# pymc-devs/pymc

Measured on AMD Instinct MI355X. Metric: effective samples/sec (and leapfrog steps/sec), 10k-param hierarchical logistic regression, one NUTS chain per GPU, higher is better.
Workload: dtype f64

## Files before the change

pymc_amd/csrc/engine.hip:

```cpp
#include <hip/hip_runtime.h>

#include <algorithm>
#include <atomic>
#include <chrono>
#include <cmath>
#include <cstdio>
#include <cstdlib>
#include <cstring>
#include <mutex>
#include <thread>
#include <utility>
#include <ctime>
#include <string>
#include <vector>

#include "kernels.h"
#include "small_kernel.h"
#include "mixture_kernel.h"
#include "nuts_mi355.h"
#include "pcg64_stream.h"
#include "advi.h"

static thread_local std::string g_err;

// ... 1185 lines not shown
  const int n = m->md.n, D = lg.D, SPAN = WAVE * m->rows_rpl;
  const int64_t n_tiles = tile0[lg.G];
  lg.ga = 1; lg.ga_w = gpw ? GB_W : W;
  lg.ga_gpw = gpw;
  lg.ga_bsz = gpw ? gpw : (lg.G + 31) / 32;
  lg.ga_flags = env_int("NUTS_GA_FLAGS", 0);
  lg.ga_T_uni = 0; lg.ga_ng_uni = 0;
  {
    bool uni = lg.G > 0;
    for (int g = 1; g < lg.G; ++g) uni = uni && (gptr[g + 1] - gptr[g] == gptr[1] - gptr[0]);
    if (uni && maxT > 0) { lg.ga_T_uni = (int32_t)maxT; lg.ga_ng_uni = gptr[1] - gptr[0]; }
  }
  lg.ga_nblk = (lg.G + lg.ga_bsz - 1) / lg.ga_bsz;
  lg.ga_auxel = n - lg.G * D;
  lg.ga_naux = m->ga_struct_ok == 2 ? (lg.ga_auxel + WAVE * lg.ga_w - 1) / (WAVE * lg.ga_w) : 0;
  lg.ga_nrec = lg.ga_nblk + lg.ga_naux;
  bool ones0 = D == 8 && env_int("NUTS_GA_ONES0", 1) != 0 && lg.N > 0;
  for (int64_t i = 0; ones0 && i < lg.N; ++i) ones0 = s->rows_X[i * D] == 1.0;
  const int DX = ones0 ? D - 1 : D;
  lg.ga_dx = DX;
  const int64_t TS = (int64_t)DX * SPAN, GA_SKEW = env_int("NUTS_GA_SKEW", DX == 7 || DX == 5 ? 1120 : 1056);
  if (GA_SKEW % DX != 0) return refuse("NUTS_GA_SKEW must be a multiple of the stored column count");
  std::vector<int64_t> coff((size_t)lg.G * W, 0);
  int64_t pos = 0, max_ct = 0;
  for (int g = 0; g < lg.G; ++g) {
    const int64_t T = tile0[g + 1] - tile0[g];
    for (int w = 0; w < W; ++w) {
      const int64_t ct = (int64_t)(w + 1) * T / W - (int64_t)w * T / W;
      coff[(size_t)g * W + w] = pos;
      pos += ct * TS + GA_SKEW;
      max_ct = std::max(max_ct, ct);
    }
  }
  lg.ga_cstride_uni = 0;
  if (lg.ga_T_uni > 0 && lg.ga_T_uni % W == 0) {
    lg.ga_cstride_uni = (lg.ga_T_uni / W) * TS + GA_SKEW;
  } else lg.ga_T_uni = 0;
  lg.Npad = n_tiles * SPAN; lg.n_spans = n_tiles;
  std::vector<double> xt((size_t)(pos + TS), 0.0);
  std::vector<int8_t> yy((size_t)(pos / DX + 2 * SPAN), 0);
  for (int g = 0; g < lg.G; ++g) {
    const int64_t T = tile0[g + 1] - tile0[g];
    for (int64_t i = gptr[g]; i < gptr[g + 1]; ++i) {
      const int64_t r = i - gptr[g], t = r / SPAN, rr = r % SPAN;
      int w = (int)(((t + 1) * W - 1) / std::max<int64_t>(T, 1));
      while (w > 0 && (int64_t)w * T / W > t) --w;
      while (w + 1 < W && (int64_t)(w + 1) * T / W <= t) ++w;
      const int64_t base = coff[(size_t)g * W + w] + (t - (int64_t)w * T / W) * TS;
      for (int d = D - DX; d < D; ++d) xt[(size_t)(base + (int64_t)(d - (D - DX)) * SPAN + rr)] = s->rows_X[i * D + d];
      yy[(size_t)(base / DX + rr)] = s->rows_y[i];
    }
  }
  lg.Xt = m->keep(dev_upload(xt.data(), xt.size()));
  lg.y = m->keep(dev_upload(yy.data(), yy.size()));
  m->rows_xt_len = (int64_t)xt.size(); m->rows_y_len = (int64_t)yy.size();
  lg.ga_coff = m->keep(dev_upload(coff.data(), coff.size()));
  lg.ga_tile0 = m->keep(dev_upload(tile0.data(), tile0.size()));
  lg.ga_part = m->keep(dev_alloc<double>((size_t)lg.G * PART_STRIDE));
  const size_t bpart_len = gpw ? 2 * (size_t)PART_STRIDE * ((lg.ga_nrec + WAVE - 1) / WAVE * WAVE) : 2 * (size_t)lg.ga_nrec * PART_STRIDE;
  lg.ga_bpart = m->keep(dev_alloc<double>(bpart_len));
  lg.ga_ticket = m->keep(dev_alloc<unsigned>(lg.ga_nblk));
  if (lg.ga_part) hipMemset(lg.ga_part, 0, (size_t)lg.G * PART_STRIDE * sizeof(double));
  if (lg.ga_bpart) hipMemset(lg.ga_bpart, 0, bpart_len * sizeof(double));
  if (lg.ga_ticket) hipMemset(lg.ga_ticket, 0, lg.ga_nblk * sizeof(unsigned));
  m->rows_grid = gpw ? lg.ga_nblk : lg.G;
  return true;
}

static bool build_rows_spans(nuts_model* m, const nuts_model_spec* s, int cus) {
  RowsDev& lg = m->md.lg;
// ... 941 lines not shown
extern "C" nuts_group* nuts_group_create(void) {
  nuts_group* g = new nuts_group();
  if (hipStreamCreateWithFlags(&g->stream, hipStreamNonBlocking) != hipSuccess) { g_err = "nuts_group_create: no stream"; delete g; return nullptr; }
  return g;
}

extern "C" int nuts_group_add(nuts_group* g, nuts_chain* c) {
  if (!g || !c || !c->m) return NUTS_E_ARG;
  nuts_model* m = c->m;
  const MvnDev& mv = m->md.mv;
  if (m->group) { g_err = "nuts_group_add: the chain's model already belongs to a group"; return NUTS_E_ARG; }
  if (m->n_chains != 1) { g_err = "nuts_group_add: a member model carries exactly one chain (its launch parity and records are the chain's)"; return NUTS_E_ARG; }
  const RowsDev& lg = m->md.lg;
  const bool is_mvn = m->md.has_mvn && (mv.aligned == 4 || mv.aligned == 8);
  const bool is_rows = m->md.has_logit && !m->md.has_mvn && lg.ga && lg.ga_naux == 0 && lg.D == 8 && m->ga_struct_ok == 1;
  const int rows_kind = lg.ga_gpw > 0 ? 3 : 2;
  if (!(is_mvn || is_rows) || c->dense || c->host_pot) {
    g_err = "nuts_group_add: chain groups advance models that are one constant-covariance MvNormal node on the row-aligned pass or the "
            "hierarchical-logit rows on the group-aligned pass (diagonal mass matrix); this chain is neither";
    return NUTS_E_ARG;
  }
  const int rows_lds = g->n == 0 ? env_int("NUTS_ROWS_GROUP_LDS", 1) : g->rows_lds;
  const int cap = g->n == 0 ? (is_rows ? ((rows_lds || rows_kind == 3) ? GAL_MAXC : GAM_MAXNC) : ((is_mvn && mv.aligned == 8 && mv.k % 16 == 0 && c->group_wide) ? GRP_MAXC : MVM_MAXC)) : g->cap;
  if (g->n >= cap) {
    g_err = cap == GRP_MAXC ? "nuts_group_add: a wide group holds at most 16 chains" : (cap == GAL_MAXC ? "nuts_group_add: a rows group holds at most 8 chains" : "nuts_group_add: a group holds at most 4 chains");
    return NUTS_E_ARG;
  }
  if (g->n > 0 && g->kind != (is_rows ? rows_kind : 1)) { g_err = "nuts_group_add: not the same model as the group's"; return NUTS_E_ARG; }
  HIPCHK(hipStreamSynchronize(m->stream));
  if (is_rows) {
    if (nuts_model* base = group_base(g)) {
      const RowsDev& bl = base->md.lg;
      if (bl.N != lg.N || bl.G != lg.G || bl.D != lg.D || bl.ga_dx != lg.ga_dx || bl.ga_w != lg.ga_w || bl.ga_gpw != lg.ga_gpw || bl.ga_nblk != lg.ga_nblk || bl.Npad != lg.Npad || bl.ga_T_uni != lg.ga_T_uni ||
          bl.ga_cstride_uni != lg.ga_cstride_uni || bl.ga_bsz != lg.ga_bsz || bl.ga_nrec != lg.ga_nrec || bl.sigma_tr != lg.sigma_tr ||
          bl.off_mu != lg.off_mu || bl.off_sigma != lg.off_sigma || bl.off_z != lg.off_z || base->md.n != m->md.n ||
          std::memcmp(&bl.z_np_mu, &lg.z_np_mu, 8 * sizeof(double)) != 0) {
        g_err = "nuts_group_add: not the same model as the group's"; return NUTS_E_ARG;
      }
      const size_t nx = (size_t)base->rows_xt_len, ny = (size_t)base->rows_y_len;
      if (nx != (size_t)m->rows_xt_len || ny != (size_t)m->rows_y_len) { g_err = "nuts_group_add: not the same model as the group's"; return NUTS_E_ARG; }
      const size_t slab = (size_t)1 << 22;
      std::vector<double> a(slab), b(slab);
      for (size_t o = 0; o < nx; o += slab) {
        const size_t k = std::min(slab, nx - o);
        HIPCHK(hipMemcpy(a.data(), bl.Xt + o, k * sizeof(double), hipMemcpyDeviceToHost));
        HIPCHK(hipMemcpy(b.data(), lg.Xt + o, k * sizeof(double), hipMemcpyDeviceToHost));
        if (std::memcmp(a.data(), b.data(), k * sizeof(double)) != 0) { g_err = "nuts_group_add: not the same model as the group's (the design matrices differ)"; return NUTS_E_ARG; }
      }
      std::vector<int8_t> ya(ny), yb(ny);
      HIPCHK(hipMemcpy(ya.data(), bl.y, ny, hipMemcpyDeviceToHost));
      HIPCHK(hipMemcpy(yb.data(), lg.y, ny, hipMemcpyDeviceToHost));
      if (std::memcmp(ya.data(), yb.data(), ny) != 0) { g_err = "nuts_group_add: not the same model as the group's (the observations differ)"; return NUTS_E_ARG; }
    }
  } else
  if (nuts_model* base = group_base(g)) {
    const MvnDev& bv = base->md.mv;
    if (bv.k != mv.k || bv.aligned != mv.aligned || bv.konst != mv.konst) { g_err = "nuts_group_add: not the same model as the group's"; return NUTS_E_ARG; }
    const size_t kk = (size_t)mv.k * mv.k;
    std::vector<double> a(kk + mv.k), b(kk + mv.k);
    HIPCHK(hipMemcpy(a.data(), bv.prec, kk * sizeof(double), hipMemcpyDeviceToHost));
    HIPCHK(hipMemcpy(b.data(), mv.prec, kk * sizeof(double), hipMemcpyDeviceToHost));
    HIPCHK(hipMemcpy(a.data() + kk, bv.mu, mv.k * sizeof(double), hipMemcpyDeviceToHost));
    HIPCHK(hipMemcpy(b.data() + kk, mv.mu, mv.k * sizeof(double), hipMemcpyDeviceToHost));
    if (std::memcmp(a.data(), b.data(), a.size() * sizeof(double)) != 0) { g_err = "nuts_group_add: not the same model as the group's (precision or mean differ)"; return NUTS_E_ARG; }
  }
  if (is_rows && (rows_lds || rows_kind == 3) && !g->gal_konst_dev) {
    HIPCHK(hipMalloc((void**)&g->gal_konst_dev, GAL_MAXC * sizeof(GalConst)));
// ... 1628 lines not shown
```

pymc_amd/csrc/model_dev.h:

```cpp
#pragma once
#include "device_math.h"
#include "nuts_mi355.h"

#define MAX_BTERMS 8
#define MAX_DERIVED 4
#define MAX_FACTOR_BT 6
#define MAX_DEFERRED 256
#define LOGIT_MAXD 8
#define SEG_MAIN_MAX 10

struct VarDev {
  int32_t offset, size, transform, deferred;
  double lower, upper;
  int32_t normal_prior;
  int32_t def_base;
  double np_mu, np_inv_var, np_lognorm;
};

struct Contrib {
  int32_t f;
  int16_t arg, slot;
  int32_t owner;
  int32_t fast;
  int32_t dist, pad;
// ... 13 lines not shown
  struct { int16_t arg, slot; int32_t bterm; } e[MAX_FACTOR_BT];
};

struct RowsDev {
  int64_t N, Npad;
  int32_t D, G;
  const double* Xt;
  const int8_t* y;
  const int64_t* gptr;
  int32_t off_mu, off_sigma, off_z, sigma_tr;
  int32_t var_mu, var_sigma, var_z, pad;
  int32_t def_mu, def_sigma;
  int32_t segK, seg_pad;
  int64_t n_spans;
  int32_t n_waves, n_seg;
  const int32_t* run_ptr;
  const int4* runs;
  const int32_t* gseg_ptr;
  double* seg_part;
  int32_t n_mixed, n_mixed_seg;
  const int64_t* mixed_span;
  const int32_t* mixed_g0;
  const int32_t* mixed_seg_base;
  const int32_t* gmix_ptr;
  double* mixed_part;
  double* wave_lp;
  int32_t ga, ga_w;
  int32_t ga_dx, ga_gpw;
  int32_t ga_nblk, ga_bsz;
  int32_t ga_T_uni, ga_flags;
  int64_t ga_ng_uni;
  const int32_t* ga_tile0;
  const int64_t* ga_coff;
  int64_t ga_cstride_uni;
  unsigned* ga_ticket;
  double* ga_part;
  double* ga_bpart;
  int32_t ga_naux, ga_nrec, ga_auxel, ga_pad2;
  double z_np_mu, z_np_inv_var, z_np_lognorm;
  double mu_c[3];
  double sg_c[2];
};

struct MvnDev {
  int32_t k, off;
  const double* mu;
  const double* prec;
  double konst;
  double* rowq;
  double* gdense;
  const double* winv; const double* winv_t;
  double* wy;
  int32_t aligned, al_nwg;
  double* al_part;
};

#define MIX_MAXK 16
struct MixDev {
  int64_t N;
  int32_t K, off_mu, off_sigma, off_w;
  int32_t tr_sigma, nwg;
  int32_t w_simplex, pad_;
  double alpha[MIX_MAXK], w_konst;
  const double* y;
  const double* assign;
  double sigma_c[MIX_MAXK], logw_c[MIX_MAXK];
  double* part;
// ... 89 lines not shown
  long long* ticks;
  int32_t tick_j;
  int32_t fdead_mode;
  int32_t* fdead;
  int32_t n_gsf, n_gs_elems;
  int32_t po_gsf, po_gslot;
  int32_t n_gs_blocks, n_orphans_b;
  double* gs_part;
  int32_t n_swf, sw_bytes, sw_rows, sw_po_leaf, sw_po_instr, sw_po_slot;
  int32_t sw_max_leaves, sw_max_slots, sw_max_instr, sw_blocks;
  const char* sw_blob;
  int32_t gs_lds_rows, gs_lds_bytes;
  double* adj;
  int32_t n_glong, glong_pad;
  const GLong* glong;
  double* adj_red;
  int32_t n_lins, n_lin_targets;
  const LinDev* lins;
  const LinTarget* lin_targets;
  const LinSrc* lin_srcs;
  double* lin_gdense;
};

#ifdef NUTS_KTIMING
__device__ __forceinline__ long long tick_now() {
  unsigned long long t;
  asm volatile("s_waitcnt vmcnt(0) lgkmcnt(0)\n\ts_memtime %0\n\ts_waitcnt lgkmcnt(0)" : "=s"(t) :: "memory");
  return (long long)t;
}
#define TICK(md, cond, slot) do { if (cond) (md).ticks[slot] = tick_now(); } while (0)
#else
#define TICK(md, cond, slot) do { } while (0)
#endif

__device__ __forceinline__ void st_agent(double* p, double v) {
  __hip_atomic_store(reinterpret_cast<unsigned long long*>(p), (unsigned long long)__double_as_longlong(v), __ATOMIC_RELAXED,
                     __HIP_MEMORY_SCOPE_AGENT);
}
__device__ __forceinline__ double ld_agent(const double* p) {
  return __longlong_as_double((long long)__hip_atomic_load(reinterpret_cast<const unsigned long long*>(p), __ATOMIC_RELAXED,
                                                           __HIP_MEMORY_SCOPE_AGENT));
}

template <int BATCH = 8>
__device__ __forceinline__ double sum_strided(const double* base, int stride, int s0, int s1) {
  double acc = 0.0;
  for (int s = s0; s < s1; s += BATCH) {
    double v[BATCH];
#pragma unroll
    for (int u = 0; u < BATCH; ++u) v[u] = base[(int64_t)min(s + u, s1 - 1) * stride];
#pragma unroll
    for (int u = 0; u < BATCH; ++u) acc += (s + u < s1) ? v[u] : 0.0;
  }
  return acc;
}

#define CTL_CHUNKS 8

__device__ __forceinline__ double deferred_finish(double gx_local, double S, double dxdq, double dj) {
  return fma(gx_local + S, dxdq, dj);
}

#define PROG_LDS_MAX 12288

struct Prog {
  const VarDev* vars;
// ... 778 lines not shown
```

pymc_amd/csrc/rows_ga_kernel.h:

```cpp
#pragma once
#include "rows_kernel.h"

__device__ __forceinline__ void ga_def_local(const RowsDev& R, bool is_mu, double qn, double& gx, double& dxdq, double& dj, double& lp) {
  if (is_mu) {
    const double r = qn - R.mu_c[0];
    const double z = r * R.mu_c[1];
    lp = -0.5 * z * z - R.mu_c[2] + (-0.91893853320467274178);
    gx = -z * R.mu_c[1]; dxdq = 1.0; dj = 0.0;
  } else {
    double x, lj;
    if (R.sigma_tr == NUTS_TR_LOG) { x = exp(qn); dxdq = x; lj = qn; dj = 1.0; }
    else { x = qn; dxdq = 1.0; lj = 0.0; dj = 0.0; }
    const double z = x * R.sg_c[0];
    double lpf = -0.5 * z * z - R.sg_c[1] + (-0.22579135264472743236);
    double g = -z * R.sg_c[0];
    if (!(x >= 0)) { lpf = -INFINITY; g = 0.0; }
    gx = g; lp = lj + lpf;
  }
}

template <int D, int RPL>
__device__ __forceinline__ void ga_load(const RowsDev& R, int64_t xoff, int lane, double (&x)[D][RPL], uint32_t& ybits) {
  constexpr int SPAN = WAVE * RPL;
  const double* tile = R.Xt + xoff + lane * RPL;
  const int8_t* yp = R.y + xoff / D + lane * RPL;
  if (RPL == 2) ybits = *reinterpret_cast<const uint16_t*>(yp);
  else ybits = *reinterpret_cast<const uint32_t*>(yp);
#pragma unroll
  for (int d = 0; d < D; ++d) {
#pragma unroll
    for (int k = 0; k < RPL; k += 2) {
      const double2 a = *reinterpret_cast<const double2*>(tile + d * SPAN + k);
      x[d][k] = a.x; x[d][k + 1] = a.y;
    }
  }
}

typedef double ga_v2d __attribute__((ext_vector_type(2)));
struct GaTileRegs { ga_v2d c[8]; uint32_t y; };

__device__ __forceinline__ void ga_issue8(const double* base , const int8_t* ybase,
                                          uint32_t voff16, uint32_t voff2, GaTileRegs& t) {
  const double* base2 = base + 512;
  asm volatile(
      "s_nop 4\n\t"
      "global_load_dwordx4 %0, %9, %10\n\t"
      "global_load_dwordx4 %1, %9, %10 offset:1024\n\t"
      "global_load_dwordx4 %2, %9, %10 offset:2048\n\t"
      "global_load_dwordx4 %3, %9, %10 offset:3072\n\t"
      "global_load_dwordx4 %4, %9, %11\n\t"
      "global_load_dwordx4 %5, %9, %11 offset:1024\n\t"
      "global_load_dwordx4 %6, %9, %11 offset:2048\n\t"
      "global_load_dwordx4 %7, %9, %11 offset:3072\n\t"
      "global_load_ushort %8, %12, %13"
      : "=&v"(t.c[0]), "=&v"(t.c[1]), "=&v"(t.c[2]), "=&v"(t.c[3]), "=&v"(t.c[4]), "=&v"(t.c[5]), "=&v"(t.c[6]), "=&v"(t.c[7]), "=&v"(t.y)
      : "v"(voff16), "s"(base), "s"(base2), "v"(voff2), "s"(ybase)
      : "memory");
}

template <int N>
__device__ __forceinline__ void ga_wait8(GaTileRegs& t) {
  asm volatile("s_waitcnt vmcnt(%9)"
               : "+v"(t.c[0]), "+v"(t.c[1]), "+v"(t.c[2]), "+v"(t.c[3]), "+v"(t.c[4]), "+v"(t.c[5]), "+v"(t.c[6]), "+v"(t.c[7]), "+v"(t.y)
               : "i"(N));
}

struct GaTileRegs7 { ga_v2d c[7]; uint32_t y; };

__device__ __forceinline__ void ga_issue8(const double* base, const int8_t* ybase, uint32_t voff16, uint32_t voff2, GaTileRegs7& t) {
  const double* base2 = base + 512;
  asm volatile(
      "s_nop 4\n\t"
      "global_load_dwordx4 %0, %8, %9\n\t"
      "global_load_dwordx4 %1, %8, %9 offset:1024\n\t"
      "global_load_dwordx4 %2, %8, %9 offset:2048\n\t"
      "global_load_dwordx4 %3, %8, %9 offset:3072\n\t"
      "global_load_dwordx4 %4, %8, %10\n\t"
      "global_load_dwordx4 %5, %8, %10 offset:1024\n\t"
      "global_load_dwordx4 %6, %8, %10 offset:2048\n\t"
      "global_load_ushort %7, %11, %12"
      : "=&v"(t.c[0]), "=&v"(t.c[1]), "=&v"(t.c[2]), "=&v"(t.c[3]), "=&v"(t.c[4]), "=&v"(t.c[5]), "=&v"(t.c[6]), "=&v"(t.y)
      : "v"(voff16), "s"(base), "s"(base2), "v"(voff2), "s"(ybase)
      : "memory");
}

template <int N>
__device__ __forceinline__ void ga_wait8(GaTileRegs7& t) {
  asm volatile("s_waitcnt vmcnt(%8)"
               : "+v"(t.c[0]), "+v"(t.c[1]), "+v"(t.c[2]), "+v"(t.c[3]), "+v"(t.c[4]), "+v"(t.c[5]), "+v"(t.c[6]), "+v"(t.y)
               : "i"(N));
}

__device__ __forceinline__ void ga_unpack(const GaTileRegs& t, double (&xx)[8][2]) {
#pragma unroll
  for (int dd = 0; dd < 8; ++dd) { xx[dd][0] = t.c[dd].x; xx[dd][1] = t.c[dd].y; }
}
__device__ __forceinline__ void ga_unpack(const GaTileRegs7& t, double (&xx)[8][2]) {
  xx[0][0] = 1.0; xx[0][1] = 1.0;
#pragma unroll
  for (int dd = 1; dd < 8; ++dd) { xx[dd][0] = t.c[dd - 1].x; xx[dd][1] = t.c[dd - 1].y; }
}
template <int DX> struct GaTileSel { typedef GaTileRegs type; };
template <> struct GaTileSel<7> { typedef GaTileRegs7 type; };

template <int D, int RPL, bool ILV = false>
__device__ __forceinline__ void ga_tile(const double (&x)[D][RPL], uint32_t yb, const double (&beta)[D], int nvalid, int lane,
                                        double (&acc)[D], double& lp) {
  if constexpr (ILV && RPL == 2) {
    double eta[2] = {0.0, 0.0}, yk[2], l[2], rr[2];
#pragma unroll
    for (int d = 0; d < D; ++d) { eta[0] = fma(x[d][0], beta[d], eta[0]); eta[1] = fma(x[d][1], beta[d], eta[1]); }
    yk[0] = (double)(yb & 0xffu); yk[1] = (double)((yb >> 8) & 0xffu);
    logit_row2(eta, yk, l, rr);
#pragma unroll
    for (int k = 0; k < 2; ++k) {
      const bool in = lane * 2 + k < nvalid;
      lp += in ? l[k] : 0.0;
      rr[k] = in ? rr[k] : 0.0;
    }
#pragma unroll
    for (int d = 0; d < D; ++d) { acc[d] = fma(rr[0], x[d][0], acc[d]); acc[d] = fma(rr[1], x[d][1], acc[d]); }
    return;
  }
// ... 38 lines not shown
__device__ __forceinline__ void ga_hyper(const ModelDev& md, const QView& qv, int fold, int par, int lane, double& hval0, double& hph0) {
  const RowsDev& R = md.lg;
  if (fold & GA_FOLD_SRC) {
    const LeanSrc prev = lean_src(md, par ^ 1);
    rows_hyper_fold_elem<D>(R, prev.part, prev.stride, prev.nblk, prev.def_loc, qv, lane, hval0, hph0);
  } else {
    const int e = lane % (2 * D);
    const int i = e < D ? R.off_mu + e : R.off_sigma + (e - D);
    if (qv.composed) { hph0 = qv.p_half(i); hval0 = fma(qv.eps, qv.var[i] * hph0, qv.q[i]); }
    else { hph0 = 0.0; hval0 = qv.q[i]; }
  }
}

template <int D, int RPL, int DX = D>
__global__ __launch_bounds__(64 * GA_MAXW, 4) void k_rows_ga(GaArgs a) {
  constexpr int SPAN = WAVE * RPL;
  static_assert(DX == D || (D == 8 && DX == 7), "only the intercept column of an 8-column model is elided");
  typedef typename GaTileSel<DX>::type Tile;
  constexpr int LOADS = DX + 1;
  const ModelDev& md = a.md;
  const ArenaDev& A = a.A;
  const EvalIO& io = a.io;
  const int j = a.j, rev = a.rev, fold = a.fold, par = a.par, d = a.d, max_depth = a.max_depth;
  const double Emax = a.Emax;
  HostStatus* const st = a.st;
  const RowsDev& R = md.lg;
  int b = (int)blockIdx.x;
  if (fold & GA_FOLD_CTL) {
    if (b == 0) { control_lean(md, A, a.cio, a.cj, a.cd, Emax, max_depth, st, a.cseq, lean_src(md, par ^ 1)); return; }
    --b;
  }
  const int g = b;
  const int tid = threadIdx.x, lane = tid & (WAVE - 1), w = __builtin_amdgcn_readfirstlane(tid >> 6), W = (int)blockDim.x >> 6;
  Leaf lf; QView qv;
  const int aborted = load_aborted(io, A);
  resolve_leaf(io, A, j, lf, qv);
  const bool leaf = io.mode != MODE_PLAIN;
  __shared__ double s_acc[GA_MAXW][2][D + 1];
  __shared__ double s_red[NDOT];
  __shared__ double s_cp[GA_MAXCHUNK][PART_STRIDE];
  __shared__ int s_info[4];
  __shared__ double s_keep[5][WAVE];
  __shared__ __attribute__((aligned(16))) char s_args[(sizeof(GaArgs) + 15) / 16 * 16];
  __shared__ __attribute__((aligned(16))) char s_auxprog[GA_AUX_PROG_LDS];
  if (b >= R.G) {
    static_assert(GA_AUX_SCRATCH_DOUBLES(GA_MAXW) <= GA_MAXCHUNK * PART_STRIDE, "auxiliary scratch does not fit the chunk buffer");
    double hv, hp;
    ga_hyper<D>(md, qv, fold, par, lane, hv, hp);
    const int aux_id = b - R.G;
    ga_aux<4>((const GaArgs*)__builtin_amdgcn_kernarg_segment_ptr(), aux_id, hv, hp, &s_cp[0][0], GA_MAXW, s_auxprog,
                R.ga_bpart + ((int64_t)par * R.ga_nrec + R.ga_nblk + aux_id) * PART_STRIDE, 1);
    return;
  }

  int T; int64_t ng, cbase;
  if (R.ga_T_uni > 0) { T = R.ga_T_uni; ng = R.ga_ng_uni; cbase = (int64_t)(g * W + w) * R.ga_cstride_uni; }
  else {
    T = __builtin_amdgcn_readfirstlane(R.ga_tile0[g + 1] - R.ga_tile0[g]);
    ng = __builtin_amdgcn_readfirstlane((int)(R.gptr[g + 1] - R.gptr[g]));
    const int64_t cb = R.ga_coff[g * W + w];
    cbase = ((int64_t)__builtin_amdgcn_readfirstlane((int)(cb >> 32)) << 32) | (uint32_t)__builtin_amdgcn_readfirstlane((int)(cb & 0xffffffffll));
  }
  const int c0 = (int)((int64_t)w * T / W), c2 = (int)((int64_t)(w + 1) * T / W);
  const int n = c2 - c0;
  const int nA = (n + 1) / 2;
  const int nsw = rev ? n - nA : nA;
  constexpr int64_t TS = (int64_t)DX * SPAN;
  auto local_at = [&](int i) { return rev ? (i < nsw ? nA + i : i - nsw) : i; };
  auto tile_at = [&](int i) { return cbase + (int64_t)local_at(i) * TS; };
  const int l_last = (c2 == T) ? n - 1 : -1;
  const int n_last = (int)(ng - (int64_t)(T - 1) * SPAN);
  double xa[D][RPL], xb[D][RPL];
  uint32_t ya = 0, yb = 0;
  Tile ta, tb;
  if constexpr (D == 8 && RPL == 2) {
    const uint32_t voff16 = (uint32_t)lane * 16u, voff2 = (uint32_t)lane * 2u;
    const int64_t o0 = tile_at(0), o1 = tile_at(min(1, max(n - 1, 0)));
    ga_issue8(R.Xt + o0, R.y + o0 / DX, voff16, voff2, ta);
    ga_issue8(R.Xt + o1, R.y + o1 / DX, voff16, voff2, tb);
  } else {
    ga_load<D, RPL>(R, tile_at(0), lane, xa, ya);
  }
  if (lane == 0) {
#pragma unroll
    for (int dd = 0; dd <= D; ++dd) { s_acc[w][0][dd] = 0.0; s_acc[w][1][dd] = 0.0; }
  }
  {
    const uint4* ka = (const uint4*)__builtin_amdgcn_kernarg_segment_ptr();
    for (int t = tid; t < (int)((sizeof(GaArgs) + 15) / 16); t += (int)blockDim.x) reinterpret_cast<uint4*>(s_args)[t] = ka[t];
  }
  __syncthreads();

  double hval0, hph0;
  ga_hyper<D>(md, qv, fold, par, lane, hval0, hph0);
  const int dl = lane % D;
  const int iz = R.off_z + g * D + dl;
  double beta[D];
  {
    double zq, zph;
    if (qv.composed) { zph = fma(qv.half, qv.g[iz], qv.p[iz]); zq = fma(qv.eps, qv.var[iz] * zph, qv.q[iz]); }
    else { zph = 0.0; zq = qv.q[iz]; }
    const double m_lane = __shfl(hval0, dl);
    const double sraw = __shfl(hval0, D + dl);
    const double s_lane = R.sigma_tr == NUTS_TR_LOG ? exp(sraw) : sraw;
    const double bl = fma(s_lane, zq, m_lane);
#pragma unroll
    for (int dd = 0; dd < D; ++dd) beta[dd] = readlane_d(bl, dd);
    if (w == 0) { s_keep[0][lane] = hval0; s_keep[1][lane] = hph0; s_keep[2][lane] = zq; s_keep[3][lane] = zph; s_keep[4][lane] = s_lane; }
  }
  if (aborted) return;

  {
    double acc[D], lp = 0.0;
#pragma unroll
    for (int dd = 0; dd < D; ++dd) acc[dd] = 0.0;
    int half = rev ? 1 : 0;
    auto flush = [&]() {
#pragma unroll
      for (int dd = 0; dd < D; ++dd) {
        const double sum = wave_sum(acc[dd]);
        if (lane == 0) s_acc[w][half][dd] = sum;
        acc[dd] = 0.0;
      }
      const double sum = wave_sum(lp);
      if (lane == 0) s_acc[w][half][D] = sum;
      lp = 0.0;
      half ^= 1;
    };
#define GA_STAGE(X, Y, I)                                                                   \
    {                                                                                        \
      if ((I) == nsw) flush();                                                               \
      ga_tile<D, RPL>(X, Y, beta, local_at(I) == l_last ? n_last : SPAN, lane, acc, lp);     \
    }
    const int nm1 = n - 1;
    if constexpr (D == 8 && RPL == 2) {
      const uint32_t voff16 = (uint32_t)lane * 16u, voff2 = (uint32_t)lane * 2u;
      auto issue = [&](int i, Tile& t) {
        const int64_t off = tile_at(min(i, nm1));
        ga_issue8(R.Xt + off, R.y + off / DX, voff16, voff2, t);
      };
#define GA_ASTAGE(T, I)                                                                      \
      {                                                                                      \
        ga_wait8<LOADS>(T);                                                                  \
        if ((I) == nsw) flush();                                                             \
        double xx[8][2];                                                                     \
        ga_unpack(T, xx);                                                                    \
        ga_tile<8, 2>(xx, T.y, beta, local_at(I) == l_last ? n_last : SPAN, lane, acc, lp); \
      }
      for (int i = 0; i < n; i += 2) {
        GA_ASTAGE(ta, i)
        if (i + 1 >= n) break;
        issue(i + 2, ta);
        GA_ASTAGE(tb, i + 1)
        issue(i + 3, tb);
      }
      ga_wait8<0>(ta); ga_wait8<0>(tb);
#undef GA_ASTAGE
    } else {
      for (int i = 0; i < n; i += 2) {
        ga_load<D, RPL>(R, tile_at(min(i + 1, nm1)), lane, xb, yb);
        GA_STAGE(xa, ya, i)
        if (i + 1 >= n) break;
        ga_load<D, RPL>(R, tile_at(min(i + 2, nm1)), lane, xa, ya);
        GA_STAGE(xb, yb, i + 1)
      }
    }
#undef GA_STAGE
    if (n > 0) flush();
  }

  ga_tail<D>(*reinterpret_cast<const GaArgs*>(s_args), g, s_acc, s_red, s_cp, s_info, s_keep);
}

template <int D>
__device__ __forceinline__ void ga_tail(const GaArgs& T, int g, double (&s_acc)[GA_MAXW][2][D + 1], double (&s_red)[NDOT],
                                        double (&s_cp)[GA_MAXCHUNK][PART_STRIDE], int (&s_info)[4], double (&s_keep)[5][WAVE]) {
  const ModelDev& md = T.md;
  const ArenaDev& A = T.A;
  const EvalIO& io = T.io;
  const RowsDev& R = md.lg;
  const int j = T.j, par = T.par, d = T.d;
  const int tid = threadIdx.x, lane = tid & (WAVE - 1), w = tid >> 6, W = (int)blockDim.x >> 6;
  Leaf lf; QView qv;
  resolve_leaf(io, A, j, lf, qv);
  const bool leaf = io.mode != MODE_PLAIN;
  const bool tree = io.mode == MODE_TREE;
  const int dl = lane % D;
  const int iz = R.off_z + g * D + dl;
  MergePrefetch mpf;
// ... 102 lines not shown
```

pymc_amd/csrc/rows_ga_multi_kernel.h:

```cpp
#pragma once
#include "mvn_multi_kernel.h"

#define GAM_MAXC 8
#define GAM_MAXNC 4

struct GaLeafArgs {
  ArenaDev A;
  EvalIO io, cio;
  double Emax;
  HostStatus* st;
  double* ga_part;
  double* ga_bpart;
  unsigned* ga_ticket;
  double* def_loc;
  int j, fold, par, d, max_depth, cj, cd, cseq;
  int slot, pad;
};

template <int NC>
struct GaMultiArgs {
  GaLeafArgs c[NC];
  int rev, pad;
};

// ... 121 lines not shown
                                         typename GaTileSel<DX>::type& t) {
  const ga_v2d* p = reinterpret_cast<const ga_v2d*>(base) + lane;
#pragma unroll
  for (int k = 0; k < DX; ++k) t.c[k] = p[k * WAVE];
  t.y = *reinterpret_cast<const uint16_t*>(ybase + 2 * lane);
}

template <int NC, int OCC, int DX>
__global__ __launch_bounds__(64 * GA_MAXW, OCC) void k_rows_ga_multi(ModelDev md, GaMultiArgs<NC> ma) {
  constexpr int D = 8, RPL = 2, SPAN = WAVE * RPL, PIPE = 2;
  typedef typename GaTileSel<DX>::type Tile;
  const RowsDev& R = md.lg;
  if ((int)blockIdx.x < GAM_MAXC) {
    int ci = -1;
#pragma unroll
    for (int c = 0; c < NC; ++c) ci = (int)blockIdx.x == ma.c[c].slot ? c : ci;
    if (ci < 0) return;
    const GaLeafArgs& L = ma.c[ci];
    if (L.fold & GA_FOLD_CTL) control_lean(md, L.A, L.cio, L.cj, L.cd, L.Emax, L.max_depth, L.st, L.cseq, gam_src(R, L, L.par ^ 1));
    return;
  }
  const int g = (int)blockIdx.x - GAM_MAXC;
  const int rev = ma.rev;
  const int tid = threadIdx.x, lane = tid & (WAVE - 1), w = __builtin_amdgcn_readfirstlane(tid >> 6), W = (int)blockDim.x >> 6;
  __shared__ double s_acc[NC][GA_MAXW][2][D + 1];
  __shared__ double s_red[NC][NDOT];
  __shared__ double s_cp[GA_MAXCHUNK][PART_STRIDE];
  __shared__ int s_info[NC][4];
  __shared__ double s_keep[NC][5][WAVE];
  __shared__ double s_beta[NC][D];
  __shared__ __attribute__((aligned(16))) char s_args[(sizeof(GaMultiArgs<NC>) + 15) / 16 * 16];

  int T; int64_t ng, cbase;
  if (R.ga_T_uni > 0) { T = R.ga_T_uni; ng = R.ga_ng_uni; cbase = (int64_t)(g * W + w) * R.ga_cstride_uni; }
  else {
    T = __builtin_amdgcn_readfirstlane(R.ga_tile0[g + 1] - R.ga_tile0[g]);
    ng = __builtin_amdgcn_readfirstlane((int)(R.gptr[g + 1] - R.gptr[g]));
    const int64_t cb = R.ga_coff[g * W + w];
    cbase = ((int64_t)__builtin_amdgcn_readfirstlane((int)(cb >> 32)) << 32) | (uint32_t)__builtin_amdgcn_readfirstlane((int)(cb & 0xffffffffll));
  }
  const int c0 = (int)((int64_t)w * T / W), c2 = (int)((int64_t)(w + 1) * T / W);
  const int n = c2 - c0;
  const int nA = (n + 1) / 2;
  const int nsw = rev ? n - nA : nA;
  constexpr int64_t TS = (int64_t)DX * SPAN;
  auto local_at = [&](int i) { return rev ? (i < nsw ? nA + i : i - nsw) : i; };
  auto tile_at = [&](int i) { return cbase + (int64_t)local_at(i) * TS; };
  const int l_last = (c2 == T) ? n - 1 : -1;
  const int n_last = (int)(ng - (int64_t)(T - 1) * SPAN);
  if (lane == 0) {
#pragma unroll
    for (int c = 0; c < NC; ++c)
#pragma unroll
      for (int dd = 0; dd <= D; ++dd) { s_acc[c][w][0][dd] = 0.0; s_acc[c][w][1][dd] = 0.0; }
  }
  {
    static_assert(alignof(GaMultiArgs<NC>) == 8 && sizeof(GaMultiArgs<NC>) % 8 == 0, "kernarg layout: the second argument follows the model at the next multiple of 8");
    const uint2* ka = (const uint2*)__builtin_amdgcn_kernarg_segment_ptr() + (sizeof(ModelDev) + 7) / 8;
    for (int t = tid; t < (int)(sizeof(GaMultiArgs<NC>) / 8); t += (int)blockDim.x) reinterpret_cast<uint2*>(s_args)[t] = ka[t];
  }

  int dead = 0;
#pragma unroll
  for (int c = 0; c < NC; ++c) dead |= load_aborted(ma.c[c].io, ma.c[c].A) ? (1 << c) : 0;
  if (dead == (1 << NC) - 1) return;
  for (int c = w; c < NC; c += W) {
    const GaLeafArgs& L = ma.c[c];
// ... 117 lines not shown
```

pymc_amd/csrc/rows_gal_kernel.h:

```cpp
#pragma once
#include "rows_ga_multi_kernel.h"

#define GAL_MAXC GAM_MAXC
#define GAL_PF 2
#define GAL_RING (GAL_PF + 1)

struct GalConst {
  ArenaDev A;
  double Emax;
  HostStatus* st;
  double* ga_part; double* ga_bpart; unsigned* ga_ticket; double* def_loc;
  int max_depth, slot;
};
struct GalLeaf {
  EvalIO io, cio;
  const double* uniforms; const double* log_uniforms;
  int j, fold, par, d, cj, cd, cseq, slot;
};
template <int NC>
struct GalArgs {
  GalLeaf c[NC];
  int rev, pad;
};

// ... 114 lines not shown
  }
  const int g = (int)blockIdx.x - GAL_MAXC;
  const int W = R.ga_w;
  __shared__ double s_acc[NC][GA_MAXW][2][D + 1];
  __shared__ int s_info[NC][4];
  __shared__ int s_dead[NC];
  __shared__ double s_keep[NC][5][2 * D];
  const uint32_t ring0 = (uint32_t)(uintptr_t)(&s_ring[0]);

  {
    GaLeafArgs* Lw = &s_L[w];
    if (lane == 0) gal_assemble(*Lw, konst[la.c[w].slot], la.c[w]);
  }
  __syncthreads();
  const GaLeafArgs& L = s_L[w];
  const int dead = load_aborted(L.io, L.A);
  if (lane == 0) {
    s_dead[w] = dead;
#pragma unroll
    for (int ww = 0; ww < GA_MAXW; ++ww)
#pragma unroll
      for (int dd = 0; dd <= D; ++dd) { s_acc[w][ww][0][dd] = 0.0; s_acc[w][ww][1][dd] = 0.0; }
  }

  int T; int64_t ng;
  if (R.ga_T_uni > 0) { T = R.ga_T_uni; ng = R.ga_ng_uni; }
  else {
    T = __builtin_amdgcn_readfirstlane(R.ga_tile0[g + 1] - R.ga_tile0[g]);
    ng = __builtin_amdgcn_readfirstlane((int)(R.gptr[g + 1] - R.gptr[g]));
  }
  const int rev = la.rev;
  const int n_last = (int)(ng - (int64_t)(T - 1) * SPAN);
  auto chunk_base = [&](int ww) -> int64_t {
    if (R.ga_T_uni > 0) return (int64_t)(g * W + ww) * R.ga_cstride_uni;
    const int64_t cb = R.ga_coff[g * W + ww];
    return ((int64_t)__builtin_amdgcn_readfirstlane((int)(cb >> 32)) << 32) | (uint32_t)__builtin_amdgcn_readfirstlane((int)(cb & 0xffffffffll));
  };
  struct It { int ww, pos, n, nA, nsw, has_last; int64_t cbase; };
  auto it_chunk = [&](It& it, int ww) {
    it.ww = ww; it.pos = 0;
    const int c0 = (int)((unsigned)ww * (unsigned)T / (unsigned)W), c2 = (int)((unsigned)(ww + 1) * (unsigned)T / (unsigned)W);
    it.n = c2 - c0; it.nA = (it.n + 1) / 2; it.nsw = rev ? it.n - it.nA : it.nA;
    it.has_last = c2 == T;
    it.cbase = ww < W ? chunk_base(ww) : 0;
  };
  auto it_skip_empty = [&](It& it) { while (it.ww < W && it.pos >= it.n) it_chunk(it, it.ww + 1); };
  auto it_local = [&](const It& it) { return rev ? (it.pos < it.nsw ? it.nA + it.pos : it.pos - it.nsw) : it.pos; };

  const uint32_t l16 = (uint32_t)lane * 16u;
  auto request = [&](const It& it, int slot) {
    const int64_t off = it.cbase + (int64_t)it_local(it) * TS;
    const double* xt = R.Xt + off;
    const int8_t* yt = R.y + off / DX;
    const uint32_t dst = ring0 + (uint32_t)slot * SLOT;
#pragma unroll
    for (int i = 0; i < LPT; ++i) {
      int k = w + i * NC;
      k = k < ITEMS ? k : 0;
      if (k < DX) gal_dma16(reinterpret_cast<const char*>(xt + (int64_t)k * SPAN) + l16, dst + (uint32_t)k * 1024u);
      else gal_dma4(yt + 4 * (lane & 31), dst + (uint32_t)DX * 1024u);
    }
  };

  It ld; it_chunk(ld, 0); it_skip_empty(ld);
  It ev = ld;
  It lastreq = ld;
#pragma unroll
// ... 113 lines not shown
```

pymc_amd/csrc/rows_gb_kernel.h:

```cpp
#pragma once
#include "rows_ga_kernel.h"

#define GB_F_EMPTY 2
#define GB_F_NOSUMS 4
#define GB_F_NOSTREAM 8
#define GB_F_NOPOST 16
#define GB_F_NOBPART 32
#define GB_F_NOCTL 64
#define GB_F_PROLOGUE 128
#ifdef NUTS_KNOCKOUT
#define GB_XF(bit) ((R.ga_flags & (bit)) != 0)
#else
#define GB_XF(bit) false
#endif
#ifndef GB_W
#define GB_W 8
#endif
#define GB_MAXGPW 16

template <int D, int DX>
__device__ __forceinline__ void gb_load(const RowsDev& R, int64_t xoff, int lane, double (&x)[D][2], uint32_t& ybits) {
  constexpr int SPAN = WAVE * 2;
  const double* tile = R.Xt + xoff + lane * 2;
  ybits = *reinterpret_cast<const uint16_t*>(R.y + xoff / DX + lane * 2);
// ... 16 lines not shown
__device__ __forceinline__ void gb_body(const ModelDev& md, const GbChain& a, int b_in, const GaArgs* karg) {
  constexpr int SPAN = WAVE * 2;
  constexpr int64_t TS = (int64_t)DX * SPAN;
  const ArenaDev& A = a.A;
  const EvalIO& io = a.io;
  const RowsDev& R = md.lg;
  const int j = a.j, fold = a.fold, par = a.par, d = a.d;
  auto src_of = [&](int pp) {
    const int npad_ = (R.ga_nrec + WAVE - 1) / WAVE * WAVE;
    return LeanSrc{a.ga_bpart + (int64_t)pp * PART_STRIDE * npad_, 1, R.ga_nrec, a.def_loc + (int64_t)pp * 4 * MAX_DEFERRED, npad_};
  };
  int b = b_in;
  if (GB_XF(GB_F_EMPTY)) return;
  if ((fold & GA_FOLD_CTL) || !karg) {
    if (b == 0 && (GB_XF(GB_F_NOCTL) || !(fold & GA_FOLD_CTL))) return;
    if (b == 0) { control_lean<8, true>(md, A, a.cio, a.cj, a.cd, a.Emax, a.max_depth, a.st, a.cseq, src_of(par ^ 1), GB_W * WAVE > VEC_THREADS ? VEC_THREADS : 0); return; }
    --b;
  }
  const int tid = threadIdx.x, lane = tid & (WAVE - 1), w = __builtin_amdgcn_readfirstlane(tid >> 6);
  const int GPW = R.ga_gpw;
  const int g0 = b * GPW, cnt = min(R.G, g0 + GPW) - g0;
  Leaf lf; QView qv;
  const int aborted = load_aborted(io, A);
  resolve_leaf(io, A, j, lf, qv);
  const bool leaf = io.mode != MODE_PLAIN, tree = io.mode == MODE_TREE;
  __shared__ double s_rec[GB_MAXGPW][PART_STRIDE];
  __shared__ double s_red[GB_W][NDOT];
  __shared__ int s_ml[2];
  __shared__ __attribute__((aligned(16))) char s_auxprog[GA_AUX_PROG_LDS];
  const bool tk = b == (int)(R.ga_nblk / 2) && tid == 0 && (md.tick_j < 0 || j == md.tick_j);
  TICK(md, tk, 0);

  auto geom = [&](int g, int& T, int& ng, int64_t& cbase) {
    if (R.ga_T_uni > 0) { T = R.ga_T_uni; ng = (int)R.ga_ng_uni; cbase = (int64_t)g * R.ga_cstride_uni; }
    else {
      T = __builtin_amdgcn_readfirstlane(R.ga_tile0[g + 1] - R.ga_tile0[g]);
      ng = __builtin_amdgcn_readfirstlane((int)(R.gptr[g + 1] - R.gptr[g]));
      const int64_t cb = R.ga_coff[g];
      cbase = ((int64_t)__builtin_amdgcn_readfirstlane((int)(cb >> 32)) << 32) | (uint32_t)__builtin_amdgcn_readfirstlane((int)(cb & 0xffffffffll));
    }
  };
  double xa[D][2];
  uint32_t ya;
  int T0, ng0; int64_t cb0;
  geom(min(g0 + w, R.G - 1), T0, ng0, cb0);
  gb_load<D, DX>(R, cb0, lane, xa, ya);

  __shared__ double s_hS[2 * D];
  const int he = lane % (2 * D);
  const bool h_mu = he < D;
  const int hi = (h_mu ? R.off_mu : R.off_sigma) + (h_mu ? he : he - D);
  double2 hl01 = make_double2(0.0, 1.0), hl23 = make_double2(0.0, 0.0);
  double hq = 0.0, hv = 0.0;
  if (fold & GA_FOLD_SRC) {
    const LeanSrc prev = src_of(par ^ 1);
    const int slot = (h_mu ? R.def_mu : R.def_sigma) + (h_mu ? he : he - D);
    hl01 = reinterpret_cast<const double2*>(prev.def_loc)[2 * slot];
    hl23 = reinterpret_cast<const double2*>(prev.def_loc)[2 * slot + 1];
    hq = qv.q[hi]; hv = qv.var[hi];
    if (GB_XF(GB_F_NOSUMS)) { if (tid < 2 * D) s_hS[tid] = 0.0; } else {
    constexpr int PERW = (2 * D + GB_W - 1) / GB_W;
    double v[PERW][SLOT_SUM_MAXR];
#pragma unroll
    for (int u = 0; u < PERW; ++u) {
      const int pe = min(w + u * GB_W, 2 * D - 1);
      const int k = pe < D ? PART_DMU + pe : PART_DSG + (pe - D);
      slot_sum_issue(prev.part + (int64_t)k * prev.slot_major, prev.slot_major, lane, v[u]);
// ... 156 lines not shown
```

Measured before the change: 18120.

## Generalize uniform chunk offsets and hoist tile loads ahead of leaf resolution

Result: no change. 18280, median of 4 (+0.9%).

```diff
diff --git a/pymc_amd/csrc/engine.hip b/pymc_amd/csrc/engine.hip
--- a/pymc_amd/csrc/engine.hip
+++ b/pymc_amd/csrc/engine.hip
@@ -1241,10 +1241,14 @@
       max_ct = std::max(max_ct, ct);
     }
   }
-  lg.ga_cstride_uni = 0;
-  if (lg.ga_T_uni > 0 && lg.ga_T_uni % W == 0) {
-    lg.ga_cstride_uni = (lg.ga_T_uni / W) * TS + GA_SKEW;
-  } else lg.ga_T_uni = 0;
+  lg.ga_gstride_uni = 0; lg.ga_skew_uni = 0;
+  if (lg.ga_T_uni > 0) {
+    if (lg.ga_T_uni >= (1 << 24)) return refuse("logit rows: group too large for the group-aligned layout");
+    lg.ga_gstride_uni = lg.ga_T_uni * TS + W * GA_SKEW; lg.ga_skew_uni = GA_SKEW;
+    for (int g = 0; g < lg.G; ++g)
+      for (int w = 0; w < W; ++w)
+        if (ga_chunk_uni(lg, g, w, W, TS) != coff[(size_t)g * W + w]) return refuse("logit rows: closed-form chunk offsets disagree with the chunk table");
+  }
   lg.Npad = n_tiles * SPAN; lg.n_spans = n_tiles;
   std::vector<double> xt((size_t)(pos + TS), 0.0);
   std::vector<int8_t> yy((size_t)(pos / DX + 2 * SPAN), 0);
@@ -2252,7 +2256,7 @@
     if (nuts_model* base = group_base(g)) {
       const RowsDev& bl = base->md.lg;
       if (bl.N != lg.N || bl.G != lg.G || bl.D != lg.D || bl.ga_dx != lg.ga_dx || bl.ga_w != lg.ga_w || bl.ga_gpw != lg.ga_gpw || bl.ga_nblk != lg.ga_nblk || bl.Npad != lg.Npad || bl.ga_T_uni != lg.ga_T_uni ||
-          bl.ga_cstride_uni != lg.ga_cstride_uni || bl.ga_bsz != lg.ga_bsz || bl.ga_nrec != lg.ga_nrec || bl.sigma_tr != lg.sigma_tr ||
+          bl.ga_gstride_uni != lg.ga_gstride_uni || bl.ga_skew_uni != lg.ga_skew_uni || bl.ga_bsz != lg.ga_bsz || bl.ga_nrec != lg.ga_nrec || bl.sigma_tr != lg.sigma_tr ||
           bl.off_mu != lg.off_mu || bl.off_sigma != lg.off_sigma || bl.off_z != lg.off_z || base->md.n != m->md.n ||
           std::memcmp(&bl.z_np_mu, &lg.z_np_mu, 8 * sizeof(double)) != 0) {
         g_err = "nuts_group_add: not the same model as the group's"; return NUTS_E_ARG;
diff --git a/pymc_amd/csrc/model_dev.h b/pymc_amd/csrc/model_dev.h
--- a/pymc_amd/csrc/model_dev.h
+++ b/pymc_amd/csrc/model_dev.h
@@ -69,7 +69,7 @@
   int64_t ga_ng_uni;
   const int32_t* ga_tile0;
   const int64_t* ga_coff;
-  int64_t ga_cstride_uni;
+  int64_t ga_gstride_uni, ga_skew_uni;
   unsigned* ga_ticket;
   double* ga_part;
   double* ga_bpart;
@@ -225,6 +225,11 @@
 #else
 #define TICK(md, cond, slot) do { } while (0)
 #endif
+
+__host__ __device__ __forceinline__ int64_t ga_chunk_uni(const RowsDev& R, int g, int w, int W, int64_t TS) {
+  const int c0 = (int)((unsigned)w * (unsigned)R.ga_T_uni / (unsigned)W);
+  return (int64_t)g * R.ga_gstride_uni + (int64_t)c0 * TS + (int64_t)w * R.ga_skew_uni;
+}
 
 __device__ __forceinline__ void st_agent(double* p, double v) {
   __hip_atomic_store(reinterpret_cast<unsigned long long*>(p), (unsigned long long)__double_as_longlong(v), __ATOMIC_RELAXED,
diff --git a/pymc_amd/csrc/rows_ga_kernel.h b/pymc_amd/csrc/rows_ga_kernel.h
--- a/pymc_amd/csrc/rows_ga_kernel.h
+++ b/pymc_amd/csrc/rows_ga_kernel.h
@@ -40,9 +40,11 @@
 struct GaTileRegs { ga_v2d c[8]; uint32_t y; };
 
 __device__ __forceinline__ void ga_issue8(const double* base , const int8_t* ybase,
-                                          uint32_t voff16, uint32_t voff2, GaTileRegs& t) {
+                                          uint32_t voff16, uint32_t voff2, GaTileRegs& t, int go) {
   const double* base2 = base + 512;
   asm volatile(
+      "s_cmp_eq_u32 %14, 0\n\t"
+      "s_cbranch_scc1 .Lga_skip_%=\n\t"
       "s_nop 4\n\t"
       "global_load_dwordx4 %0, %9, %10\n\t"
       "global_load_dwordx4 %1, %9, %10 offset:1024\n\t"
@@ -52,24 +54,32 @@
       "global_load_dwordx4 %5, %9, %11 offset:1024\n\t"
       "global_load_dwordx4 %6, %9, %11 offset:2048\n\t"
       "global_load_dwordx4 %7, %9, %11 offset:3072\n\t"
-      "global_load_ushort %8, %12, %13"
+      "global_load_ushort %8, %12, %13\n"
+      ".Lga_skip_%=:"
       : "=&v"(t.c[0]), "=&v"(t.c[1]), "=&v"(t.c[2]), "=&v"(t.c[3]), "=&v"(t.c[4]), "=&v"(t.c[5]), "=&v"(t.c[6]), "=&v"(t.c[7]), "=&v"(t.y)
-      : "v"(voff16), "s"(base), "s"(base2), "v"(voff2), "s"(ybase)
-      : "memory");
+      : "v"(voff16), "s"(base), "s"(base2), "v"(voff2), "s"(ybase), "s"(__builtin_amdgcn_readfirstlane(go))
+      : "memory", "scc");
 }
 
 template <int N>
-__device__ __forceinline__ void ga_wait8(GaTileRegs& t) {
-  asm volatile("s_waitcnt vmcnt(%9)"
+__device__ __forceinline__ void ga_wait8(GaTileRegs& t, int younger) {
+  asm volatile("s_cmp_lg_u32 %10, 0\n\t"
+               "s_cbranch_scc1 .Lga_cnt_%=\n\t"
+               "s_waitcnt vmcnt(0)\n"
+               ".Lga_cnt_%=:\n\t"
+               "s_waitcnt vmcnt(%9)"
                : "+v"(t.c[0]), "+v"(t.c[1]), "+v"(t.c[2]), "+v"(t.c[3]), "+v"(t.c[4]), "+v"(t.c[5]), "+v"(t.c[6]), "+v"(t.c[7]), "+v"(t.y)
-               : "i"(N));
+               : "i"(N), "s"(__builtin_amdgcn_readfirstlane(younger))
+               : "scc");
 }
 
 struct GaTileRegs7 { ga_v2d c[7]; uint32_t y; };
 
-__device__ __forceinline__ void ga_issue8(const double* base, const int8_t* ybase, uint32_t voff16, uint32_t voff2, GaTileRegs7& t) {
+__device__ __forceinline__ void ga_issue8(const double* base, const int8_t* ybase, uint32_t voff16, uint32_t voff2, GaTileRegs7& t, int go) {
   const double* base2 = base + 512;
   asm volatile(
+      "s_cmp_eq_u32 %13, 0\n\t"
+      "s_cbranch_scc1 .Lga_skip_%=\n\t"
       "s_nop 4\n\t"
       "global_load_dwordx4 %0, %8, %9\n\t"
       "global_load_dwordx4 %1, %8, %9 offset:1024\n\t"
@@ -78,17 +88,23 @@
       "global_load_dwordx4 %4, %8, %10\n\t"
       "global_load_dwordx4 %5, %8, %10 offset:1024\n\t"
       "global_load_dwordx4 %6, %8, %10 offset:2048\n\t"
-      "global_load_ushort %7, %11, %12"
+      "global_load_ushort %7, %11, %12\n"
+      ".Lga_skip_%=:"
       : "=&v"(t.c[0]), "=&v"(t.c[1]), "=&v"(t.c[2]), "=&v"(t.c[3]), "=&v"(t.c[4]), "=&v"(t.c[5]), "=&v"(t.c[6]), "=&v"(t.y)
-      : "v"(voff16), "s"(base), "s"(base2), "v"(voff2), "s"(ybase)
-      : "memory");
+      : "v"(voff16), "s"(base), "s"(base2), "v"(voff2), "s"(ybase), "s"(__builtin_amdgcn_readfirstlane(go))
+      : "memory", "scc");
 }
 
 template <int N>
-__device__ __forceinline__ void ga_wait8(GaTileRegs7& t) {
-  asm volatile("s_waitcnt vmcnt(%8)"
+__device__ __forceinline__ void ga_wait8(GaTileRegs7& t, int younger) {
+  asm volatile("s_cmp_lg_u32 %9, 0\n\t"
+               "s_cbranch_scc1 .Lga_cnt_%=\n\t"
+               "s_waitcnt vmcnt(0)\n"
+               ".Lga_cnt_%=:\n\t"
+               "s_waitcnt vmcnt(%8)"
                : "+v"(t.c[0]), "+v"(t.c[1]), "+v"(t.c[2]), "+v"(t.c[3]), "+v"(t.c[4]), "+v"(t.c[5]), "+v"(t.c[6]), "+v"(t.y)
-               : "i"(N));
+               : "i"(N), "s"(__builtin_amdgcn_readfirstlane(younger))
+               : "scc");
 }
 
 __device__ __forceinline__ void ga_unpack(const GaTileRegs& t, double (&xx)[8][2]) {
@@ -193,10 +209,6 @@
   }
   const int g = b;
   const int tid = threadIdx.x, lane = tid & (WAVE - 1), w = __builtin_amdgcn_readfirstlane(tid >> 6), W = (int)blockDim.x >> 6;
-  Leaf lf; QView qv;
-  const int aborted = load_aborted(io, A);
-  resolve_leaf(io, A, j, lf, qv);
-  const bool leaf = io.mode != MODE_PLAIN;
   __shared__ double s_acc[GA_MAXW][2][D + 1];
   __shared__ double s_red[NDOT];
   __shared__ double s_cp[GA_MAXCHUNK][PART_STRIDE];
@@ -206,6 +218,8 @@
   __shared__ __attribute__((aligned(16))) char s_auxprog[GA_AUX_PROG_LDS];
   if (b >= R.G) {
     static_assert(GA_AUX_SCRATCH_DOUBLES(GA_MAXW) <= GA_MAXCHUNK * PART_STRIDE, "auxiliary scratch does not fit the chunk buffer");
+    Leaf lf; QView qv;
+    resolve_leaf(io, A, j, lf, qv);
     double hv, hp;
     ga_hyper<D>(md, qv, fold, par, lane, hv, hp);
     const int aux_id = b - R.G;
@@ -214,19 +228,19 @@
     return;
   }
 
+  constexpr int64_t TS = (int64_t)DX * SPAN;
   int T; int64_t ng, cbase;
-  if (R.ga_T_uni > 0) { T = R.ga_T_uni; ng = R.ga_ng_uni; cbase = (int64_t)(g * W + w) * R.ga_cstride_uni; }
+  if (R.ga_T_uni > 0) { T = R.ga_T_uni; ng = R.ga_ng_uni; cbase = ga_chunk_uni(R, g, w, W, TS); }
   else {
     T = __builtin_amdgcn_readfirstlane(R.ga_tile0[g + 1] - R.ga_tile0[g]);
     ng = __builtin_amdgcn_readfirstlane((int)(R.gptr[g + 1] - R.gptr[g]));
     const int64_t cb = R.ga_coff[g * W + w];
     cbase = ((int64_t)__builtin_amdgcn_readfirstlane((int)(cb >> 32)) << 32) | (uint32_t)__builtin_amdgcn_readfirstlane((int)(cb & 0xffffffffll));
   }
-  const int c0 = (int)((int64_t)w * T / W), c2 = (int)((int64_t)(w + 1) * T / W);
+  const int c0 = (int)((unsigned)w * (unsigned)T / (unsigned)W), c2 = (int)((unsigned)(w + 1) * (unsigned)T / (unsigned)W);
   const int n = c2 - c0;
   const int nA = (n + 1) / 2;
   const int nsw = rev ? n - nA : nA;
-  constexpr int64_t TS = (int64_t)DX * SPAN;
   auto local_at = [&](int i) { return rev ? (i < nsw ? nA + i : i - nsw) : i; };
   auto tile_at = [&](int i) { return cbase + (int64_t)local_at(i) * TS; };
   const int l_last = (c2 == T) ? n - 1 : -1;
@@ -234,14 +248,23 @@
   double xa[D][RPL], xb[D][RPL];
   uint32_t ya = 0, yb = 0;
   Tile ta, tb;
+  const uint32_t voff2 = (uint32_t)lane * 2u;
+  auto issue = [&](int i, Tile& t) {
+    const int l = local_at(min(i, max(n - 1, 0)));
+    const int64_t off = cbase + (int64_t)l * TS;
+    const uint32_t v2 = voff2 < (uint32_t)(l == l_last ? n_last : SPAN) ? voff2 : 0u;
+    ga_issue8(R.Xt + off, R.y + off / DX, v2 * 8u, v2, t, (i < n || i == 0) ? 1 : 0);
+  };
   if constexpr (D == 8 && RPL == 2) {
-    const uint32_t voff16 = (uint32_t)lane * 16u, voff2 = (uint32_t)lane * 2u;
-    const int64_t o0 = tile_at(0), o1 = tile_at(min(1, max(n - 1, 0)));
-    ga_issue8(R.Xt + o0, R.y + o0 / DX, voff16, voff2, ta);
-    ga_issue8(R.Xt + o1, R.y + o1 / DX, voff16, voff2, tb);
+    issue(0, ta);
+    issue(1, tb);
   } else {
     ga_load<D, RPL>(R, tile_at(0), lane, xa, ya);
   }
+  Leaf lf; QView qv;
+  const int aborted = load_aborted(io, A);
+  resolve_leaf(io, A, j, lf, qv);
+  const bool leaf = io.mode != MODE_PLAIN;
   if (lane == 0) {
 #pragma unroll
     for (int dd = 0; dd <= D; ++dd) { s_acc[w][0][dd] = 0.0; s_acc[w][1][dd] = 0.0; }
@@ -295,27 +318,22 @@
     }
     const int nm1 = n - 1;
     if constexpr (D == 8 && RPL == 2) {
-      const uint32_t voff16 = (uint32_t)lane * 16u, voff2 = (uint32_t)lane * 2u;
-      auto issue = [&](int i, Tile& t) {
-        const int64_t off = tile_at(min(i, nm1));
-        ga_issue8(R.Xt + off, R.y + off / DX, voff16, voff2, t);
-      };
-#define GA_ASTAGE(T, I)                                                                      \
+#define GA_ASTAGE(T, I, YOUNGER)                                                             \
       {                                                                                      \
-        ga_wait8<LOADS>(T);                                                                  \
+        ga_wait8<LOADS>(T, (YOUNGER) ? 1 : 0);                                               \
         if ((I) == nsw) flush();                                                             \
         double xx[8][2];                                                                     \
         ga_unpack(T, xx);                                                                    \
         ga_tile<8, 2>(xx, T.y, beta, local_at(I) == l_last ? n_last : SPAN, lane, acc, lp); \
       }
+      if (n == 0) ga_wait8<0>(ta, 0);
       for (int i = 0; i < n; i += 2) {
-        GA_ASTAGE(ta, i)
+        GA_ASTAGE(ta, i, i + 1 < n)
         if (i + 1 >= n) break;
         issue(i + 2, ta);
-        GA_ASTAGE(tb, i + 1)
+        GA_ASTAGE(tb, i + 1, i + 2 < n)
         issue(i + 3, tb);
       }
-      ga_wait8<0>(ta); ga_wait8<0>(tb);
 #undef GA_ASTAGE
     } else {
       for (int i = 0; i < n; i += 2) {
diff --git a/pymc_amd/csrc/rows_ga_multi_kernel.h b/pymc_amd/csrc/rows_ga_multi_kernel.h
--- a/pymc_amd/csrc/rows_ga_multi_kernel.h
+++ b/pymc_amd/csrc/rows_ga_multi_kernel.h
@@ -177,7 +177,7 @@
   __shared__ __attribute__((aligned(16))) char s_args[(sizeof(GaMultiArgs<NC>) + 15) / 16 * 16];
 
   int T; int64_t ng, cbase;
-  if (R.ga_T_uni > 0) { T = R.ga_T_uni; ng = R.ga_ng_uni; cbase = (int64_t)(g * W + w) * R.ga_cstride_uni; }
+  if (R.ga_T_uni > 0) { T = R.ga_T_uni; ng = R.ga_ng_uni; cbase = ga_chunk_uni(R, g, w, W, (int64_t)DX * SPAN); }
   else {
     T = __builtin_amdgcn_readfirstlane(R.ga_tile0[g + 1] - R.ga_tile0[g]);
     ng = __builtin_amdgcn_readfirstlane((int)(R.gptr[g + 1] - R.gptr[g]));
diff --git a/pymc_amd/csrc/rows_gal_kernel.h b/pymc_amd/csrc/rows_gal_kernel.h
--- a/pymc_amd/csrc/rows_gal_kernel.h
+++ b/pymc_amd/csrc/rows_gal_kernel.h
@@ -170,7 +170,7 @@
   const int rev = la.rev;
   const int n_last = (int)(ng - (int64_t)(T - 1) * SPAN);
   auto chunk_base = [&](int ww) -> int64_t {
-    if (R.ga_T_uni > 0) return (int64_t)(g * W + ww) * R.ga_cstride_uni;
+    if (R.ga_T_uni > 0) return ga_chunk_uni(R, g, ww, W, TS);
     const int64_t cb = R.ga_coff[g * W + ww];
     return ((int64_t)__builtin_amdgcn_readfirstlane((int)(cb >> 32)) << 32) | (uint32_t)__builtin_amdgcn_readfirstlane((int)(cb & 0xffffffffll));
   };
diff --git a/pymc_amd/csrc/rows_gb_kernel.h b/pymc_amd/csrc/rows_gb_kernel.h
--- a/pymc_amd/csrc/rows_gb_kernel.h
+++ b/pymc_amd/csrc/rows_gb_kernel.h
@@ -72,7 +72,7 @@
   TICK(md, tk, 0);
 
   auto geom = [&](int g, int& T, int& ng, int64_t& cbase) {
-    if (R.ga_T_uni > 0) { T = R.ga_T_uni; ng = (int)R.ga_ng_uni; cbase = (int64_t)g * R.ga_cstride_uni; }
+    if (R.ga_T_uni > 0) { T = R.ga_T_uni; ng = (int)R.ga_ng_uni; cbase = ga_chunk_uni(R, g, 0, 1, TS); }
     else {
       T = __builtin_amdgcn_readfirstlane(R.ga_tile0[g + 1] - R.ga_tile0[g]);
       ng = __builtin_amdgcn_readfirstlane((int)(R.gptr[g + 1] - R.gptr[g]));
```
